# Immortalqx/pi-slam-fusion

Hardware: AMD Instinct MI355X
Metric: keyframes/sec fused (4000x3000 -> 256^2 tiles, 5-band) (higher is better)
Workload: dtype f32; 1 GPU; cfg-2/cfg-A: 4000x3000 BGR8 keyframes, serpentine sortie, Map2D.Scale=1, 5-band Laplacian, CV_32FC3 (ForceFloat=1) pyramids, frames resident in HBM; frames_per_rank=2646, sortie_frames_before_timing=20, lookahead=48, rendered_rank0=2666, culled_tiles_rank0=490117

## Files before the change

pi-slam-fusion_amd/csrc/kernels.hip:

```cpp
#include "kernels.hpp"
#include "warp_index.hpp"
#include "env.hpp"
#include <climits>
#include <cmath>
#include <cstdlib>
#include <type_traits>

#ifndef PF_EXPERIMENTS
#define PF_EXPERIMENTS 0
#endif
#ifndef PF_ROWTAB
#define PF_ROWTAB 0
#endif
#ifndef PF_HYBRID_W
#define PF_HYBRID_W 0
#endif

namespace pf {

constexpr bool kExp = PF_EXPERIMENTS != 0;

__device__ __forceinline__ double clamp_int_range(double v)
{
    v = (v < (double)INT_MAX) ? v : (double)INT_MAX;
// ... 718 lines not shown
        if (X < vec_w) {
            float a = r0.w + r4.w;
            const float bb = (r1.w + r3.w) + r2.w;
            a = a + (r2.w + r2.w);
            o.w = (a + bb * 4.f) * (1.f / 256);
        } else
            o.w = (r2.w * 6 + (r1.w + r3.w) * 4 + r0.w + r4.w) * (1.f / 256);
        if constexpr (!F32) o.pad = 0;
        Bt[p][q] = o;
        if (p >= 1 && p < LQH - 1 && q >= 1 && q < LQW - 1) {
            if (g.write_next) gw_out[(long)Y * ncols + X] = o;
            if (g.top_select) select_store<F32>(lay.top_lap_off, lay.top_w_off, g.level + 1, table, g.tiles_x, X, Y, o.c, o.w);
        }
    }
    lds_barrier();
    if (kExp && (g.ablate & 4)) return;
    Hx (*U)[LBW] = reinterpret_cast<Hx (*)[LBW]>(&Ht[0][0]);
    static_assert(sizeof(Hx) * LQH * LBW <= sizeof(Hx) * LAH * LQW, "U must fit in Ht");
    const bool edge = (x0 == 0) || (x0 + LBW >= g.cols) || (ncols == 1);
    for (int idx = tid; idx < LQH * LBW; idx += LNT) {
        const int p = idx >> 6, lx = idx & 63;
        const int x = x0 + lx, sx = x >> 1, j = (lx >> 1) + 1;
        Hx u;
        if (!edge) {
            const Px a = Bt[p][j - 1], b = Bt[p][j], c = Bt[p][j + 1];
#pragma unroll
            for (int k = 0; k < 3; k++) u.c[k] = up_h_val<WT, false>((WT)a.c[k], (WT)b.c[k], (WT)c.c[k], x & 1, false, false, false);
        } else {
            const bool one = ncols == 1, le = sx == 0, re = sx == ncols - 1;
            const Px a = Bt[p][(le && !F32) ? (one ? j : j + 1) : j - 1], b = Bt[p][j], c = Bt[p][(re && !F32) ? j : j + 1];
#pragma unroll
            for (int k = 0; k < 3; k++) {
                if constexpr (F32) u.c[k] = up_h_val<WT, true>(a.c[k], b.c[k], c.c[k], x & 1, le, re, one);
                else u.c[k] = up_h_val<WT, false>((WT)a.c[k], (WT)b.c[k], (WT)c.c[k], x & 1, false, false, false);
            }
        }
        u.w = 0.f;
        U[p][lx] = u;
    }
    lds_barrier();
#pragma unroll
    for (int it = 0; it < ND; it++) {
        const uint64_t ent = ents[it];
        if (!ent) continue;
        const int idx = tid + it * LNT, ly = idx >> 6, lx = idx & 63;
        const int y = y0 + ly, x = x0 + lx;
        const Px gpx = A[ly + 4][lx + 4];
        if (!(gpx.w >= dwv[it])) continue;
        const uint64_t slot = ent & ~(uint64_t)1;
        const int loc = (y & (ts - 1)) * ts + (x & (ts - 1));
        const int sy = y >> 1;
        int syn = sy + 1; if (syn >= nrows) syn = nrows - 1;
        int syp = sy - 1; if (syp < 0) syp = nrows > 1 ? 1 : 0;
        const Hx u1 = U[sy - by0][lx], u2 = U[syn - by0][lx];
        T out[3];
        if (y & 1) {
#pragma unroll
            for (int k = 0; k < 3; k++) out[k] = sat_sub(gpx.c[k], cast_up((u1.c[k] + u2.c[k]) * 4));
        } else {
            const Hx u0 = U[syp - by0][lx];
#pragma unroll
            for (int k = 0; k < 3; k++) out[k] = sat_sub(gpx.c[k], cast_up(u0.c[k] + u1.c[k] * 6 + u2.c[k]));
        }
        T PF_GLOBAL* dl = (T PF_GLOBAL*)(slot + lay.lap_off) + loc * 3;
        dl[0] = out[0]; dl[1] = out[1]; dl[2] = out[2];
        ((float PF_GLOBAL*)(slot + lay.w_off))[loc] = gpx.w;
    }
    if (st + 1 < LS) {
        lds_barrier();
        Px keep;
        const bool mv = tid < 7 * LAW;
        if (mv) keep = (&A[0][0])[LBH * LAW + tid];
        lds_barrier();
        if (mv) (&A[0][0])[tid] = keep;
    }
    }
}

__device__ __forceinline__ void phase_stamp(unsigned long long* st, int slot)
{
    if (st) {
        unsigned long long t;
        asm volatile("s_memtime %0\n\ts_waitcnt lgkmcnt(0)" : "=s"(t) :: "memory");
        if (threadIdx.x == 0) st[slot] = t;
    }
}

__device__ unsigned long long g_select_seen[kMaxLevels], g_select_won[kMaxLevels];

constexpr int kPatchBytes = 81920 - 44928;

template <bool F32, int LBH, int LNT, bool STAMP = false, int ILP = 2, bool PATCH = false, bool WA = false, class LO = LevelOffsets, class GA = LevelArgs>
__device__ __forceinline__ void level3_block(const bool FROM_WARP, const LO& lay, const GA& g, const FusedWarp& wa,
                                             const uint8_t* __restrict__ src, const PxT<F32>* __restrict__ gw_in,
                                             PxT<F32>* __restrict__ gw_out, const uint64_t* __restrict__ table_generic, const int b,
                                             unsigned long long* stamps = nullptr, const uint64_t* tab0 = nullptr)
{
    const uint64_t PF_GLOBAL* __restrict__ table = (const uint64_t PF_GLOBAL*)table_generic;
    if (STAMP) phase_stamp(stamps, 0);
    struct StampExit { unsigned long long* st; __device__ StampExit(unsigned long long* p) : st(p) {} __device__ ~StampExit() { asm volatile("s_waitcnt vmcnt(0)" ::: "memory"); phase_stamp(st, 5); } };
    struct NoExit { __device__ NoExit(unsigned long long*) {} };
    typename std::conditional<STAMP, StampExit, NoExit>::type at_exit(stamps);
    (void)at_exit;
    using T = typename Pix<F32>::T; using WT = typename Pix<F32>::WT;
    using Px = PxT<F32>;
    constexpr int LAH = LBH + 7, LQH = LBH / 2 + 2;
    static_assert(LNT >= 32 * (LBH / 2), "one thread per 2x2 output quad (threads beyond that help in stages A and B only)");
    struct Bx { T c[F32 ? 3 : 4]; };
    constexpr int kPitch = LBH == 24 ? LAW : 2 * LAWH;
    __shared__ Px A[LAH][kPitch];
    constexpr int kTail = PATCH ? kPatchBytes : (int)(sizeof(Bx) * LQH * LQW);
    static_assert(kTail >= (int)(sizeof(Bx) * LQH * LQW), "Bt must fit");
    __shared__ __attribute__((aligned(16))) unsigned char tail[kTail];
    Bx (*Bt)[LQW] = reinterpret_cast<Bx (*)[LQW]>(tail);
    auto Aat = [&](int r, int c) -> Px& { return A[r][(c & 1) * LAWH + (c >> 1)]; };
    static_assert(LBH != 32 || PATCH || sizeof(A) + sizeof(tail) <= (F32 ? 42 : 32) * 1280, "LDS budget (64x32 blocks)");
    static_assert(LBH != 24 || sizeof(A) + sizeof(tail) <= 32 * 1280, "LDS budget (64x24 blocks: four workgroups per CU for both pyramid types)");
    static_assert(LBH != 32 || !PATCH || sizeof(A) + sizeof(tail) <= 64 * 1280, "LDS budget (64x32 blocks with a source patch: two per CU)");
    static_assert(LBH != 64 || sizeof(A) + sizeof(tail) <= (F32 ? 128 : 64) * 1280, "LDS budget (64x64 blocks of 1024 threads: int16 two per CU, fp32 one)");

    int bx, by; block_xy(g, b, bx, by);
    const int x0 = g.cx0 + bx * LBW, y0 = g.cy0 + by * LBH;
    const int ax0 = x0 - 4, ay0 = y0 - 4;
    const int nrows = g.rows >> 1, ncols = g.cols >> 1;
    const int bx0 = (x0 >> 1) - 1, by0 = (y0 >> 1) - 1;
    const int tid = threadIdx.x;
    const int sh = 8 - g.level, ts = kElePixels >> g.level;
    if (kExp && (g.ablate & 512) && !FROM_WARP) __builtin_amdgcn_s_setprio(2);

    const int qx = tid & 31, qy = tid >> 5;
    const int dx0 = x0 + 2 * qx, dy0 = y0 + 2 * qy;
    uint64_t ent = 0;
    if (tid < 32 * (LBH / 2) && dx0 < g.cols && dy0 < g.rows) {
        const int ti = (dy0 >> sh) * g.tiles_x + (dx0 >> sh);
        if (tab0) ent = ((const uint64_t PF_GLOBAL*)tab0)[ti];
        else ent = table[ti];
        if (sh >= 3) { if (cell_culled(ent, dx0, dy0, ts, sh)) ent = 0; }
        else {
            bool all = true;
#pragma unroll
            for (int k = 0; k < 4; k++) all = all && cell_culled(ent, dx0 + (k & 1), dy0 + (k >> 1), ts, sh);
            if (all) ent = 0;
        }
        ent &= ~kEntCells;
    }

    if (kExp && FROM_WARP && (g.ablate & 1024) && tid >= LNT / 2) __builtin_amdgcn_s_setprio(1);
    if (kExp && FROM_WARP && (g.ablate & 2048) && tid < LNT / 2) __builtin_amdgcn_s_setprio(1);
    if (FROM_WARP) {
        const bool inner = ax0 >= 0 && ax0 + LAW <= g.cols && ay0 >= 0 && ay0 + LAH <= g.rows;
        constexpr int RS = LNT / LAW;
        const int r0 = tid / LAW, c = tid - r0 * LAW;
        const bool near101 = g.rows >= 8 && g.cols >= 8;
        auto col_of = [&](int cc) {
            int x = ax0 + cc;
            if (!inner) x = near101 ? border_reflect101_near(x, g.cols) : border_reflect101(x, g.cols);
            return x;
        };
        auto row_of = [&](int r) {
            int y = ay0 + r;
            if (!inner) y = near101 ? border_reflect101_near(y, g.rows) : border_reflect101(y, g.rows);
            return y;
        };
        if constexpr (PATCH) {
            const float fxc = (float)(ax0 + LAW / 2), fyc = (float)(ay0 + LAH / 2);
            const float Wc = wa.Mf[6] * fxc + wa.Mf[7] * fyc + wa.Mf[8], iw = __builtin_amdgcn_rcpf(Wc);
            const float pcx = (wa.Mf[0] * fxc + wa.Mf[1] * fyc + wa.Mf[2]) * iw, pcy = (wa.Mf[3] * fxc + wa.Mf[4] * fyc + wa.Mf[5]) * iw;
            const int icx = (int)__builtin_floorf(fminf(fmaxf(pcx, -1.0e6f), 1.0e6f)), icy = (int)__builtin_floorf(fminf(fmaxf(pcy, -1.0e6f), 1.0e6f));
            int px0 = __builtin_amdgcn_readfirstlane(icx) - wa.phx, py0 = __builtin_amdgcn_readfirstlane(icy) - wa.phy;
            int px1 = px0 + 2 * wa.phx + 2, py1 = py0 + 2 * wa.phy + 2;
            px0 = px0 > 0 ? px0 : 0; py0 = py0 > 0 ? py0 : 0;
            px1 = px1 < wa.scols ? px1 : wa.scols; py1 = py1 < wa.srows ? py1 : wa.srows;
            const int pw = px1 - px0, ph = py1 - py0;
            const int cn = wa.cn, pitch_i = wa.pitch_i, pitch_w = wa.pitch_w;
            const int sb = (px0 * cn) & ~15, sbo = px0 * cn - sb;
            const int wb = (px0 * 4) & ~15, swo = px0 * 4 - wb;
            unsigned char* const pimg = tail;
            unsigned char* const pwgt = tail + (2 * wa.phy + 2) * pitch_i;
            if (pw > 1 && ph > 1) {
                typedef uint32_t u4 __attribute__((ext_vector_type(4)));
                typedef uint32_t u4u __attribute__((ext_vector_type(4), aligned(1)));
                const int lane = tid & 63, wv = tid >> 6, nci = pitch_i >> 4;
                const bool isw = lane >= nci;
                const int ch = isw ? lane - nci : lane;
                const bool on = ch * 16 < (isw ? swo + pw * 4 : sbo + (pw - 2) * cn + 8);
                constexpr int NW = LNT / 64, UNR = 4;
                for (int rb = wv; rb < ph; rb += NW * UNR) {
                    u4 v[UNR];
#pragma unroll
                    for (int u = 0; u < UNR; u++) {
                        const int r = rb + u * NW;
                        v[u] = u4{ 0, 0, 0, 0 };
                        if (on && r < ph) {
                            if (isw) {
                                const char* rowp = (const char*)(wa.wmap + (size_t)(py0 + r) * wa.scols) + wb;
                                v[u] = *(const u4u*)(rowp + ch * 16);
                            } else {
                                const long off = (long)(py0 + r) * wa.sstep + sb + ch * 16;
                                if (off + 16 <= wa.total) v[u] = *(const u4u*)(src + off);
                                else {
                                    uint32_t w4[4] = { 0, 0, 0, 0 };
                                    for (int k = 0; k < 16; k++) if (off + k < wa.total) w4[k >> 2] |= (uint32_t)src[off + k] << (8 * (k & 3));
                                    v[u] = u4{ w4[0], w4[1], w4[2], w4[3] };
                                }
                            }
                        }
                    }
#pragma unroll
                    for (int u = 0; u < UNR; u++) {
                        const int r = rb + u * NW;
                        if (on && r < ph) *(u4*)((isw ? pwgt + r * pitch_w : pimg + r * pitch_i) + ch * 16) = v[u];
                    }
                }
            }
            __syncthreads();
            if (r0 < RS) {
                const int x = col_of(c);
                const WarpCol col = warp_col(wa, x);
                const uint32_t hisel = cn == 3 ? 0x06050403u : 0x07060504u;
                typedef uint32_t u2 __attribute__((ext_vector_type(2), aligned(1)));
                struct Cd { int X, Y, Xn, Yn; bool ok; };
                const unsigned okw = pw > 1 && ph > 1 ? (unsigned)(pw - 1) : 0u, okh = pw > 1 && ph > 1 ? (unsigned)(ph - 1) : 0u;
                auto coords = [&](int y) {
                    const double X0 = col.m0xb + wa.M[1] * y + wa.M[2], Y0 = col.m3xb + wa.M[4] * y + wa.M[5], W0 = col.m6xb + wa.M[7] * y + wa.M[8];
                    const double W = W0 + col.m6x1, xn = X0 + col.m0x1, yn = Y0 + col.m3x1;
                    const double Wn = rcp_mid_range(W);
                    const double pxn = xn * Wn, pyn = yn * Wn;
                    constexpr double kMagic = 6755399441055744.0;
                    Cd o;
                    o.Xn = (int)(uint32_t)(unsigned long long)__double_as_longlong(pxn + kMagic);
                    o.Yn = (int)(uint32_t)(unsigned long long)__double_as_longlong(pyn + kMagic);
                    o.X  = (int)(uint32_t)(unsigned long long)__double_as_longlong(pxn * 32. + kMagic);
                    o.Y  = (int)(uint32_t)(unsigned long long)__double_as_longlong(pyn * 32. + kMagic);
                    o.ok = (unsigned)((o.X >> 5) - px0) < okw && (unsigned)((o.Y >> 5) - py0) < okh;
                    return o;
                };
                auto fast = [&](const Cd& q) {
                    const int la = __mul24((q.Y >> 5) - py0, pitch_i) + __mul24(q.X >> 5, cn) - sb;
                    const u2 b0 = *(const u2*)(pimg + la), b1 = *(const u2*)(pimg + la + pitch_i);
                    const float wv_ = *(const float*)(pwgt + __mul24(q.Yn - py0, pitch_w) + q.Xn * 4 - wb);
                    PxT<F32> o;
                    o.w = wv_;
                    const float fx = (float)(q.X & 31) * (1.f / 32), fy = (float)(q.Y & 31) * (1.f / 32);
                    const float c0 = (1.f - fy) * (1.f - fx), c1 = (1.f - fy) * fx, c2 = fy * (1.f - fx), c3 = fy * fx;
                    const uint32_t h0 = __builtin_amdgcn_perm(b0.y, b0.x, hisel), h1 = __builtin_amdgcn_perm(b1.y, b1.x, hisel);
#pragma unroll
                    for (int k = 0; k < 3; k++) {
                        float v0 = (float)((b0.x >> (8 * k)) & 0xff), v1 = (float)((h0 >> (8 * k)) & 0xff);
                        float v2 = (float)((b1.x >> (8 * k)) & 0xff), v3 = (float)((h1 >> (8 * k)) & 0xff);
                        if constexpr (F32) {
                            const float sc = (float)(1. / 255.);
                            v0 = v0 * sc; v1 = v1 * sc; v2 = v2 * sc; v3 = v3 * sc;
                            o.c[k] = v0 * c0 + v1 * c1 + v2 * c2 + v3 * c3;
                        } else {
                            const float tt = __builtin_fmaf(v3, c3, __builtin_fmaf(v2, c2, __builtin_fmaf(v1, c1, v0 * c0)));
                            o.c[k] = (short)sat_short(__float2int_rn(tt));
                        }
                    }
                    if constexpr (!F32) o.pad = 0;
                    return o;
                };
                for (int r = r0; r < LAH; r += 2 * RS) {
                    const int rb = r + RS;
                    const bool hasb = rb < LAH;
                    const int y = row_of(r), yb = row_of(hasb ? rb : r);
                    if (kExp && (g.ablate & 1)) { Px z{}; z.w = (float)(x + y); Aat(r, c) = z; if (hasb) Aat(rb, c) = z; continue; }
                    const Cd qa = coords(y), qb = coords(yb);
                    if (__builtin_amdgcn_ballot_w64(!(qa.ok && qb.ok)) == 0) {
                        Aat(r, c) = fast(qa);
                        const PxT<F32> pb = fast(qb);
                        if (hasb) Aat(rb, c) = pb;
                    } else {
                        Aat(r, c) = warp_pixel<F32>(src, wa, col, y);
                        if (hasb) Aat(rb, c) = warp_pixel<F32>(src, wa, col, yb);
                    }
                }
            }
        } else
        if (ILP == 0 && WA && inner && wa.plain && block_maps_inside(wa, ax0, ay0, LAW, LAH)) {
            constexpr bool kRowTab = PF_ROWTAB != 0;
            double (*rowtab)[3][4] = reinterpret_cast<double (*)[3][4]>(tail);
            const int xb0 = ax0 & ~63;
            if constexpr (kRowTab) {
                static_assert(!kRowTab || sizeof(double) * LAH * 3 * 4 <= (size_t)kTail, "row table fits behind A");
                if (tid < LAH * 9) {
                    const int r = tid / 9, e = tid - r * 9, kx = e / 3, w = e - kx * 3;
                    const double xb = (double)(xb0 + 64 * kx), y = (double)(ay0 + r);
                    rowtab[r][kx][w] = wa.M[3 * w] * xb + wa.M[3 * w + 1] * y + wa.M[3 * w + 2];
                }
                lds_barrier();
            }
            if (r0 < RS) {
                constexpr int NR = (LAH + RS - 1) / RS;
                typedef uint32_t u2 __attribute__((ext_vector_type(2), aligned(1)));
                using p2 = typename std::conditional<F32, park8, park4>::type;
                const WarpCol col = warp_col(wa, ax0 + c);
                const int cn = wa.cn, sstep = wa.sstep;
                constexpr int CH = (F32 && LBH != 24) ? NR : (NR + 1) / 2;
                u2 b0[CH], b1[CH];
                float wq[(CH + 1) / 2] = {};
                const int rbase = r0 * NR;
                const bool seed = kExp && wa.seed_ok != 0;
                double Wn = 0.0;
#pragma unroll
                for (int h = 0; h < NR; h += CH) {
#pragma unroll
                    for (int k = h; k < h + CH && k < NR; k++) {
                        const bool has = rbase + k < LAH;
                        if (k >= LAH - (RS - 1) * NR && __builtin_amdgcn_ballot_w64(has) == 0) continue;
                        const int r = has ? rbase + k : rbase;
                        const int y = ay0 + r;
                        double X0, Y0, W0;
                        if constexpr (kRowTab) {
                            const double* t = rowtab[r][(((ax0 + c) & ~63) - xb0) >> 6];
                            X0 = t[0]; Y0 = t[1]; W0 = t[2];
                        } else {
                            X0 = col.m0xb + wa.M[1] * y + wa.M[2]; Y0 = col.m3xb + wa.M[4] * y + wa.M[5]; W0 = col.m6xb + wa.M[7] * y + wa.M[8];
                        }
                        const double W = W0 + col.m6x1, xn = X0 + col.m0x1, yn = Y0 + col.m3x1;
                        Wn = (k > 0 && seed) ? rcp_seeded(W, Wn) : rcp_mid_range(W);
                        const double pxn = xn * Wn, pyn = yn * Wn;
                        constexpr double kMagic = 6755399441055744.0;
                        const int Xn = (int)(uint32_t)(unsigned long long)__double_as_longlong(pxn + kMagic);
                        const int Yn = (int)(uint32_t)(unsigned long long)__double_as_longlong(pyn + kMagic);
                        const int X = (int)(uint32_t)(unsigned long long)__double_as_longlong(__builtin_fma(pxn, 32., kMagic));
                        const int Y = (int)(uint32_t)(unsigned long long)__double_as_longlong(__builtin_fma(pyn, 32., kMagic));
                        constexpr bool kHyb = PF_HYBRID_W != 0; const bool gw_row = kHyb && (k & 1);
                        float wgt;
                        if (gw_row) wgt = *(const float*)((const char*)wa.wmap + ((uint32_t)(__mul24(Yn, wa.scols) + Xn) << 2));
                        else wgt = radial_weight(wa, Xn, Yn);
                        const uint32_t off0 = (uint32_t)(__mul24(Y >> 5, sstep) + __mul24(cn, X >> 5));
                        if (gw_row) wq[(k - h) >> 1] = wgt;
                        if (has) *reinterpret_cast<p2*>(&Aat(r, c)) = p2{ (uint32_t)((X & 31) | (Y & 31) << 5), __float_as_uint(gw_row ? 0.f : wgt) };
                        b0[k - h] = PF_LOAD_SRC((const u2*)(src + off0)); b1[k - h] = PF_LOAD_SRC((const u2*)(src + off0 + (uint32_t)sstep));
                    }
#pragma unroll
                    for (int k = h; k < h + CH && k < NR; k++) {
                        const bool has = rbase + k < LAH;
                        if (k >= LAH - (RS - 1) * NR && __builtin_amdgcn_ballot_w64(has) == 0) continue;
                        if (!has) continue;
                        const int r = rbase + k;
                        const p2 pk = *reinterpret_cast<const p2*>(&Aat(r, c));
                        constexpr bool kHyb = PF_HYBRID_W != 0; const bool gw_row = kHyb && (k & 1);
                        Aat(r, c) = warp_finish_fast<F32>(b0[k - h].x, b0[k - h].y, b1[k - h].x, b1[k - h].y, (int)(pk.x & 31u), (int)(pk.x >> 5), gw_row ? wq[(k - h) >> 1] : __uint_as_float(pk.y), cn);
                    }
                }
            }
        } else
        if (r0 < RS) {
            const int x = col_of(c);
            const WarpCol col = warp_col(wa, x);
            if constexpr (ILP == 3) {
                for (int r = r0; r < LAH; r += 3 * RS) {
                    const int rb = r + RS, rc = r + 2 * RS;
                    const bool hasb = rb < LAH, hasc = rc < LAH;
                    const int y = row_of(r), yb = row_of(hasb ? rb : r), yc = row_of(hasc ? rc : r);
                    if (kExp && (g.ablate & 1)) { Px z{}; z.w = (float)(x + y); Aat(r, c) = z; if (hasb) Aat(rb, c) = z; if (hasc) Aat(rc, c) = z; continue; }
                    const WarpTaps ta = warp_fetch<WA>(src, wa, col, y);
                    const WarpTaps tb = warp_fetch<WA>(src, wa, col, yb);
                    if (__builtin_amdgcn_ballot_w64(hasc) != 0) {
                        const WarpTaps tc = warp_fetch<WA>(src, wa, col, yc);
                        Aat(r, c) = warp_finish<F32>(ta, wa.cn);
                        if (hasb) Aat(rb, c) = warp_finish<F32>(tb, wa.cn);
                        if (hasc) Aat(rc, c) = warp_finish<F32>(tc, wa.cn);
                    } else {
                        Aat(r, c) = warp_finish<F32>(ta, wa.cn);
                        if (hasb) Aat(rb, c) = warp_finish<F32>(tb, wa.cn);
                    }
                }
            } else
            for (int r = r0; r < LAH; r += 2 * RS) {
                const int rb = r + RS;
                const bool hasb = rb < LAH;
                int y = ay0 + r, yb = ay0 + rb;
                if (!inner) {
                    if (near101) { y = border_reflect101_near(y, g.rows); yb = border_reflect101_near(yb, g.rows); }
                    else { y = border_reflect101(y, g.rows); yb = border_reflect101(yb, g.rows); }
                }
                if (kExp && (g.ablate & 1)) { Px z{}; z.w = (float)(x + y); Aat(r, c) = z; if (hasb) Aat(rb, c) = z; continue; }
                const WarpTaps ta = warp_fetch<WA>(src, wa, col, y);
                if (__builtin_amdgcn_ballot_w64(hasb) != 0) {
                    const WarpTaps tb = warp_fetch<WA>(src, wa, col, hasb ? yb : y);
                    Aat(r, c) = warp_finish<F32>(ta, wa.cn);
                    if (hasb) Aat(rb, c) = warp_finish<F32>(tb, wa.cn);
                } else
                    Aat(r, c) = warp_finish<F32>(ta, wa.cn);
            }
        }
    } else {
        stage_from_hbm<F32, LAH, LNT, true, kPitch>(&A[0][0], gw_in, ax0, ay0, g.rows, g.cols, tid, 0, kExp && !F32 && (g.ablate & 4096));
    }
    if (STAMP) phase_stamp(stamps, 1);
    if (kExp && FROM_WARP && (g.ablate & (1024 | 2048))) __builtin_amdgcn_s_setprio(0);
    lds_barrier();
    if (STAMP) phase_stamp(stamps, 2);
    if (kExp && (g.ablate & 2)) return;
    if (!kExp && g.level < 0) return;
    if (kExp && (g.ablate & 256)) __builtin_amdgcn_s_setprio(2);

    float dwv[2][2] = { { -1.f, -1.f }, { -1.f, -1.f } };
    const uint64_t slot = ent & ~kEntLow;
    const int loc0 = (dy0 & (ts - 1)) * ts + (dx0 & (ts - 1));
    if (ent && !(ent & 1)) {
        const float PF_GLOBAL* wp = (const float PF_GLOBAL*)(slot + lay.w_off) + loc0;
#pragma unroll
        for (int j = 0; j < 2; j++) {
            typedef float f2 __attribute__((ext_vector_type(2)));
            const f2 v = PF_LOAD_W((const f2 PF_GLOBAL*)(wp + j * ts));
            dwv[j][0] = v.x; dwv[j][1] = v.y;
        }
    }
    if (sh < 3 && ent) {
        const int ti = (dy0 >> sh) * g.tiles_x + (dx0 >> sh);
        const uint64_t e2 = tab0 ? ((const uint64_t PF_GLOBAL*)tab0)[ti] : table[ti];
#pragma unroll
        for (int k = 0; k < 4; k++)
            if (cell_culled(e2, dx0 + (k & 1), dy0 + (k >> 1), ts, sh)) dwv[k >> 1][k & 1] = __builtin_nanf("");
    }

    const int vec_img = (ncols * 3 / 8) * 8, vec_w = (ncols / 8) * 8;
    static_assert((LQH / 2) * LQW <= LNT, "one B item per thread at most");
    for (int idx = tid - (LNT - (LQH / 2) * LQW); idx >= 0 && idx < (LQH / 2) * LQW; idx += LNT) {
        const int pp = idx / LQW, q = idx - pp * LQW;
        const int X = bx0 + q;
        if (X < 0 || X >= ncols) continue;
        if constexpr (F32) {
            f2 hl[7], hh[7];
            const bool vec_all = X * 3 + 2 < vec_img && X < vec_w;
            const bool uni = __builtin_amdgcn_ballot_w64(!vec_all) == 0;
            auto emit = [&](int e) {
                const int p = 2 * pp + e, Y = by0 + p;
                if (Y < 0 || Y >= nrows) return;
                Px o;
                if (uni) {
                    auto vsum = [](f2 r0, f2 r1, f2 r2, f2 r3, f2 r4) {
                        f2 a = r0 + r4;
                        const f2 bb = (r1 + r3) + r2;
                        a = a + (r2 + r2);
                        return (a + bb * 4.f) * (1.f / 256);
                    };
                    const f2 ol = vsum(hl[2 * e], hl[2 * e + 1], hl[2 * e + 2], hl[2 * e + 3], hl[2 * e + 4]);
                    const f2 oh = vsum(hh[2 * e], hh[2 * e + 1], hh[2 * e + 2], hh[2 * e + 3], hh[2 * e + 4]);
                    o.c[0] = ol.x; o.c[1] = ol.y; o.c[2] = oh.x; o.w = oh.y;
                } else {
                    float out[4];
#pragma unroll
                    for (int k = 0; k < 4; k++) {
                        auto at = [&](int j) { return k < 2 ? hl[j][k] : hh[j][k - 2]; };
                        const float r0 = at(2 * e), r1 = at(2 * e + 1), r2 = at(2 * e + 2), r3 = at(2 * e + 3), r4 = at(2 * e + 4);
                        if (k < 3 ? X * 3 + k < vec_img : X < vec_w) {
                            float a = r0 + r4;
                            const float bb = (r1 + r3) + r2;
                            a = a + (r2 + r2);
                            out[k] = (a + bb * 4.f) * (1.f / 256);
                        } else
                            out[k] = (r2 * 6 + (r1 + r3) * 4 + r0 + r4) * (1.f / 256);
                    }
                    o.c[0] = out[0]; o.c[1] = out[1]; o.c[2] = out[2]; o.w = out[3];
                }
                {
                    Bx ob; ob.c[0] = o.c[0]; ob.c[1] = o.c[1]; ob.c[2] = o.c[2];
                    Bt[p][q] = ob;
                }
                if (p >= 1 && p < LQH - 1 && q >= 1 && q < LQW - 1) {
                    if (g.write_next) gw_out[(long)Y * ncols + X] = o;
                    if (g.top_select) select_store<F32>(lay.top_lap_off, lay.top_w_off, g.level + 1, table, g.tiles_x, X, Y, o.c, o.w);
                }
            };
#pragma unroll
            for (int j = 0; j < 7; j++) {
                const f4* ev = (const f4*)&A[4 * pp + j][q]; const f4* od = (const f4*)&A[4 * pp + j][LAWH + q];
                const f4 a0 = ev[0], a1 = od[0], a2 = ev[1], a3 = od[1], a4 = ev[2];
                hl[j] = a2.xy * 6.f + (a1.xy + a3.xy) * 4.f + a0.xy + a4.xy;
                hh[j] = a2.zw * 6.f + (a1.zw + a3.zw) * 4.f + a0.zw + a4.zw;
                asm volatile("" : "+v"(hl[j]), "+v"(hh[j]) :: "memory");
                if (j == 4) emit(0);
                if (j == 6) emit(1);
            }
        } else {
            us2 h01[7], h2p[7]; float hw[7];
            auto emit = [&](int e) {
                const int p = 2 * pp + e, Y = by0 + p;
                if (Y < 0 || Y >= nrows) return;
                Px o;
                {
                    const us2 v01 = h01[2 * e + 2] * (us2)6 + (h01[2 * e + 1] + h01[2 * e + 3]) * (us2)4 + h01[2 * e] + h01[2 * e + 4];
                    const us2 v2p = h2p[2 * e + 2] * (us2)6 + (h2p[2 * e + 1] + h2p[2 * e + 3]) * (us2)4 + h2p[2 * e] + h2p[2 * e + 4];
                    const us2 o01 = (v01 + (us2)128) >> (us2)8, o2p = (v2p + (us2)128) >> (us2)8;
                    o.c[0] = (short)o01.x; o.c[1] = (short)o01.y; o.c[2] = (short)o2p.x;
                }
                {
                    const float r0 = hw[2 * e], r1 = hw[2 * e + 1], r2 = hw[2 * e + 2], r3 = hw[2 * e + 3], r4 = hw[2 * e + 4];
                    if (X < vec_w) {
                        float a = r0 + r4;
                        const float bb = (r1 + r3) + r2;
                        a = a + (r2 + r2);
                        o.w = (a + bb * 4.f) * (1.f / 256);
                    } else
                        o.w = (r2 * 6 + (r1 + r3) * 4 + r0 + r4) * (1.f / 256);
                }
                o.pad = 0;
                {
                    Bx ob; ob.c[0] = o.c[0]; ob.c[1] = o.c[1]; ob.c[2] = o.c[2]; ob.c[3] = 0;
                    Bt[p][q] = ob;
                }
                if (p >= 1 && p < LQH - 1 && q >= 1 && q < LQW - 1) {
                    if (kExp && (g.ablate & 4096)) {
                        typedef uint32_t u2g __attribute__((ext_vector_type(2)));
                        u2g v; __builtin_memcpy(&v, &o, 8);
                        if (g.write_next) ((u2g*)gw_out)[(long)Y * ncols + X] = v;
                    } else
                    if (g.write_next) gw_out[(long)Y * ncols + X] = o;
                    if (g.top_select) select_store<F32>(lay.top_lap_off, lay.top_w_off, g.level + 1, table, g.tiles_x, X, Y, o.c, o.w);
                }
            };
#pragma unroll
            for (int j = 0; j < 7; j++) {
                const PxP* ev = reinterpret_cast<const PxP*>(&A[4 * pp + j][q]); const PxP* od = reinterpret_cast<const PxP*>(&A[4 * pp + j][LAWH + q]);
                const PxP a0 = ev[0], a1 = od[0], a2 = ev[1], a3 = od[1], a4 = ev[2];
                h01[j] = a2.c01 * (us2)6 + (a1.c01 + a3.c01) * (us2)4 + a0.c01 + a4.c01;
                h2p[j] = a2.c2p * (us2)6 + (a1.c2p + a3.c2p) * (us2)4 + a0.c2p + a4.c2p;
                hw[j] = a2.w * 6 + (a1.w + a3.w) * 4 + a0.w + a4.w;
                asm volatile("" : "+v"(h01[j]), "+v"(h2p[j]), "+v"(hw[j]) :: "memory");
                if (j == 4) emit(0);
                if (j == 6) emit(1);
            }
        }
    }
    if (STAMP) phase_stamp(stamps, 3);
    lds_barrier();
    if (STAMP) phase_stamp(stamps, 4);
    if (kExp && (g.ablate & 4)) return;

    if (!ent) return;
    int ry = dy0;
    asm volatile("" : "+v"(ry));
    ry -= y0;
    const Px g00 = A[ry + 4][qx + 2], g01 = A[ry + 4][LAWH + qx + 2];
    const Px g10 = A[ry + 5][qx + 2], g11 = A[ry + 5][LAWH + qx + 2];
    const bool in01 = dx0 + 1 < g.cols, in10 = dy0 + 1 < g.rows;
    const bool s00 = g00.w >= dwv[0][0], s01 = in01 && g01.w >= dwv[0][1];
    const bool s10 = in10 && g10.w >= dwv[1][0], s11 = in10 && in01 && g11.w >= dwv[1][1];
#ifdef PF_COUNT_WINS
    if constexpr (STAMP) {
        atomicAdd(&g_select_seen[g.level], (unsigned long long)(1 + (int)in01 + (int)in10 + (int)(in10 && in01)));
        atomicAdd(&g_select_won[g.level], (unsigned long long)((int)s00 + (int)s01 + (int)s10 + (int)s11));
    }
#endif
    if (!(s00 || s01 || s10 || s11)) return;
    const int sy = dy0 >> 1, sx = dx0 >> 1;
    int syn = sy + 1; if (syn >= nrows) syn = nrows - 1;
    int syp = sy - 1; if (syp < 0) syp = nrows > 1 ? 1 : 0;
    const bool one = ncols == 1, le = sx == 0, re = sx == ncols - 1;
    const bool edge = le || re;
    const int j = qx + 1;
    const int ja = (le && !F32) ? (one ? j : j + 1) : j - 1, jc = (re && !F32) ? j : j + 1;
    const int rows3[3] = { syp - by0, sy - by0, syn - by0 };
    T PF_GLOBAL* dl = (T PF_GLOBAL*)(slot + lay.lap_off) + loc0 * 3;
    float PF_GLOBAL* dw = (float PF_GLOBAL*)(slot + lay.w_off) + loc0;
    if constexpr (F32) {
        if (__builtin_amdgcn_ballot_w64(edge) == 0) {
            f2 heL[3], hoL[3]; float he2[3], ho2[3];
#pragma unroll
            for (int r = 0; r < 3; r++) {
                const float* pa = Bt[rows3[r]][j - 1].c; const float* pb = Bt[rows3[r]][j].c; const float* pc = Bt[rows3[r]][j + 1].c;
                const f2 aL = { pa[0], pa[1] }, bL = { pb[0], pb[1] }, cL = { pc[0], pc[1] };
                const float a2 = pa[2], b2 = pb[2], c2 = pc[2];
                heL[r] = aL + bL * 6.f + cL; hoL[r] = (bL + cL) * 4.f;
                he2[r] = a2 + b2 * 6 + c2;   ho2[r] = (b2 + c2) * 4;
            }
            const f2 g00L = { g00.c[0], g00.c[1] }, g01L = { g01.c[0], g01.c[1] }, g10L = { g10.c[0], g10.c[1] }, g11L = { g11.c[0], g11.c[1] };
            const f2 o00L = g00L - (heL[0] + heL[1] * 6.f + heL[2]) * (1.f / 64);
            const f2 o01L = g01L - (hoL[0] + hoL[1] * 6.f + hoL[2]) * (1.f / 64);
            const f2 o10L = g10L - ((heL[1] + heL[2]) * 4.f) * (1.f / 64);
            const f2 o11L = g11L - ((hoL[1] + hoL[2]) * 4.f) * (1.f / 64);
            const float o00c = g00.c[2] - (he2[0] + he2[1] * 6 + he2[2]) * (1.f / 64);
            const float o01c = g01.c[2] - (ho2[0] + ho2[1] * 6 + ho2[2]) * (1.f / 64);
            const float o10c = g10.c[2] - ((he2[1] + he2[2]) * 4) * (1.f / 64);
            const float o11c = g11.c[2] - ((ho2[1] + ho2[2]) * 4) * (1.f / 64);
            auto st3 = [&](T PF_GLOBAL* p, float a, float b, float c2) { PF_STORE(p, a); PF_STORE(p + 1, b); PF_STORE(p + 2, c2); };
            if (s00) { st3(dl, o00L.x, o00L.y, o00c); PF_STORE_W(&dw[0], g00.w); }
            if (s01) { st3(dl + 3, o01L.x, o01L.y, o01c); PF_STORE_W(&dw[1], g01.w); }
            if (s10) { st3(dl + 3 * ts, o10L.x, o10L.y, o10c); PF_STORE_W(&dw[ts], g10.w); }
            if (s11) { st3(dl + 3 * ts + 3, o11L.x, o11L.y, o11c); PF_STORE_W(&dw[ts + 1], g11.w); }
            return;
        }
    }
    if constexpr (!F32) {
        ss2 he01[3], ho01[3], he2p[3], ho2p[3];
#pragma unroll
        for (int r = 0; r < 3; r++) {
            const BxP a = *reinterpret_cast<const BxP*>(&Bt[rows3[r]][ja]), bq = *reinterpret_cast<const BxP*>(&Bt[rows3[r]][j]),
                      c = *reinterpret_cast<const BxP*>(&Bt[rows3[r]][jc]);
            he01[r] = a.c01 + bq.c01 * (ss2)6 + c.c01; ho01[r] = (bq.c01 + c.c01) * (ss2)4;
            he2p[r] = a.c2p + bq.c2p * (ss2)6 + c.c2p; ho2p[r] = (bq.c2p + c.c2p) * (ss2)4;
        }
        auto up_e = [](ss2 u0, ss2 u1, ss2 u2) { return (u0 + u1 * (ss2)6 + u2 + (ss2)32) >> (ss2)6; };
        auto up_o = [](ss2 u1, ss2 u2) { return ((u1 + u2) * (ss2)4 + (ss2)32) >> (ss2)6; };
        auto px2 = [](const Px& q, ss2& c01, ss2& c2p) { const PxP& v = reinterpret_cast<const PxP&>(q); c01 = (ss2)v.c01; c2p = (ss2)v.c2p; };
        ss2 a01, a2p;
        auto st3p = [&](T PF_GLOBAL* p, ss2 c01, ss2 c2p) { PF_STORE(p, c01.x); PF_STORE(p + 1, c01.y); PF_STORE(p + 2, c2p.x); };
        if (s00) { px2(g00, a01, a2p); st3p(dl, a01 - up_e(he01[0], he01[1], he01[2]), a2p - up_e(he2p[0], he2p[1], he2p[2])); PF_STORE_W(&dw[0], g00.w); }
        if (s01) { px2(g01, a01, a2p); st3p(dl + 3, a01 - up_e(ho01[0], ho01[1], ho01[2]), a2p - up_e(ho2p[0], ho2p[1], ho2p[2])); PF_STORE_W(&dw[1], g01.w); }
        if (s10) { px2(g10, a01, a2p); st3p(dl + 3 * ts, a01 - up_o(he01[1], he01[2]), a2p - up_o(he2p[1], he2p[2])); PF_STORE_W(&dw[ts], g10.w); }
        if (s11) { px2(g11, a01, a2p); st3p(dl + 3 * ts + 3, a01 - up_o(ho01[1], ho01[2]), a2p - up_o(ho2p[1], ho2p[2])); PF_STORE_W(&dw[ts + 1], g11.w); }
        return;
    }
    WT he[3][3], ho[3][3];
#pragma unroll
    for (int r = 0; r < 3; r++) {
// ... 864 lines not shown
```

Measured before the change: 27840 keyframes/s.

## Software-pipeline warp coordinate computation with weight evaluation across rows

```diff
diff --git a/pi-slam-fusion_amd/csrc/kernels.hip b/pi-slam-fusion_amd/csrc/kernels.hip
--- a/pi-slam-fusion_amd/csrc/kernels.hip
+++ b/pi-slam-fusion_amd/csrc/kernels.hip
@@ -1044,10 +1044,77 @@
                 const int rbase = r0 * NR;
                 const bool seed = kExp && wa.seed_ok != 0;
                 double Wn = 0.0;
+                constexpr int kAll = LAH - (RS - 1) * NR;
+                constexpr bool kPipe = F32 && CH == NR && !kRowTab && PF_HYBRID_W == 0 && kAll >= 1;
+                bool piped = false;
+                if constexpr (kPipe) if (!seed) {
+                    piped = true;
+                    static_assert(kAll <= NR, "only the last thread row runs past the tile");
+                    constexpr double kMagic = 6755399441055744.0;
+                    struct Crd { int Xn, Yn, X, Y; };
+                    double k32 = 32.; asm volatile("" : "+s"(k32));
+                    auto row_at = [&](int k) { return (k < kAll || rbase + k < LAH) ? rbase + k : rbase; };
+                    auto step = [&](int k, const Crd& cur, Crd& nxt, const bool W, const bool C) {
+                        uint32_t frac = 0; float dy = 0.f, dx = 0.f, dis = 0.f, s = 0.f, sd = 0.f, su = 0.f, ed = 0.f, eu = 0.f, q0 = 0.f, t = 0.f, q = 0.f;
+                        double m1 = 0., m4 = 0., m7 = 0., Wk = 1., xn = 0., yn = 0., r = 0., e = 0., pxn = 0., pyn = 0.;
+                        if (W) {
+                            const uint32_t off0 = (uint32_t)(__mul24(cur.Y >> 5, sstep) + __mul24(cn, cur.X >> 5));
+                            b0[k] = PF_LOAD_SRC((const u2*)(src + off0)); b1[k] = PF_LOAD_SRC((const u2*)(src + (uint32_t)(off0 + (uint32_t)sstep)));
+                            frac = (uint32_t)((cur.X & 31) | (cur.Y & 31) << 5);
+                            dy = (float)cur.Yn - wa.wyc; dx = (float)cur.Xn - wa.wxc;
+                        }
+                        if (C) { const int y = ay0 + row_at(k + 1); m1 = wa.M[1] * y; m4 = wa.M[4] * y; m7 = wa.M[7] * y; }
+                        if (W && C) asm volatile("" : "+v"(m7), "+v"(dy));
+                        if (W) { dis = __builtin_fmaf(dx, dx, dy * dy); s = __builtin_amdgcn_sqrtf(dis); }
+                        if (C) {
+                            const double X0 = col.m0xb + m1 + wa.M[2], Y0 = col.m3xb + m4 + wa.M[5], W0 = col.m6xb + m7 + wa.M[8];
+                            Wk = W0 + col.m6x1; xn = X0 + col.m0x1; yn = Y0 + col.m3x1;
+                        }
+                        if (W && C) asm volatile("" : "+v"(Wk), "+v"(s));
+                        if (W) {
+                            sd = __int_as_float(__float_as_int(s) - 1); su = __int_as_float(__float_as_int(s) + 1);
+                            ed = __builtin_fmaf(-sd, s, dis); eu = __builtin_fmaf(-su, s, dis);
+                        }
+                        if (C) r = __builtin_amdgcn_rcp(Wk);
+                        if (W && C) asm volatile("" : "+v"(r), "+v"(ed), "+v"(eu));
+                        if (W) { s = ed <= 0.f ? sd : s; s = eu > 0.f ? su : s; }
+                        if (C) { e = __builtin_fma(-Wk, r, 1.0); r = __builtin_fma(r, e, r); }
+                        if (W && C) asm volatile("" : "+v"(r), "+v"(s));
+                        if (W) { q0 = s * wa.wrcp; t = __builtin_fmaf(-q0, wa.wdmax, s); }
+                        if (C) { e = __builtin_fma(-Wk, r, 1.0); r = __builtin_fma(r, e, r); }
+                        if (W && C) asm volatile("" : "+v"(r), "+v"(t));
+                        if (W) q = __builtin_fmaf(t, wa.wrcp, q0);
+                        if (C) { const double rem = __builtin_fma(-Wk, r, 1.0); r = __builtin_fma(rem, r, r); }
+                        if (W && C) asm volatile("" : "+v"(r), "+v"(q));
+                        if (W) {
+                            float w = 1.f - q;
+                            if (wa.wtype != 0) w = w * w;
+                            w = fmaxf(w, 1e-5f);
+                            *reinterpret_cast<p2*>(&Aat(row_at(k), c)) = p2{ frac, __float_as_uint(w) };
+                        }
+                        if (C) {
+                            pxn = xn * r; pyn = yn * r;
+                            nxt.Xn = (int)(uint32_t)(unsigned long long)__double_as_longlong(pxn + kMagic);
+                            nxt.Yn = (int)(uint32_t)(unsigned long long)__double_as_longlong(pyn + kMagic);
+                            nxt.X = (int)(uint32_t)(unsigned long long)__double_as_longlong(__builtin_fma(pxn, k32, kMagic));
+                            nxt.Y = (int)(uint32_t)(unsigned long long)__double_as_longlong(__builtin_fma(pyn, k32, kMagic));
+                        }
+                    };
+                    Crd qa{}, qb{};
+                    step(-1, qa, qb, false, true); qa = qb;
+#pragma unroll
+                    for (int k = 0; k < kAll - 1; k++) { step(k, qa, qb, true, true); qa = qb; }
+                    if (kAll == NR || __builtin_amdgcn_ballot_w64(rbase + kAll < LAH) == 0) step(kAll - 1, qa, qb, true, false);
+                    else {
+#pragma unroll
+                        for (int k = kAll - 1; k < NR - 1; k++) { step(k, qa, qb, true, true); qa = qb; }
+                        step(NR - 1, qa, qb, true, false);
+                    }
+                }
 #pragma unroll
                 for (int h = 0; h < NR; h += CH) {
 #pragma unroll
-                    for (int k = h; k < h + CH && k < NR; k++) {
+                    for (int k = h; k < h + CH && k < NR && !piped; k++) {
                         const bool has = rbase + k < LAH;
                         if (k >= LAH - (RS - 1) * NR && __builtin_amdgcn_ballot_w64(has) == 0) continue;
                         const int r = has ? rbase + k : rbase;
```

Result: no change. 28320 keyframes/s, median of 6 (+1.7%).
